# RVC-Project/obs-rvc

Measured on AMD Instinct MI355X. Metric: audio frames/sec (10 ms hops of new input, 160 ms chunks @16 kHz), higher is better.
Workload: dtype f32; 1 GPU; BASELINE configs[1]: 1 stream(s)/GPU, ContentVec v2-768 + RMVPE + NSF-HiFiGAN v2-48k, retrieval off, preset full; streams_per_gpu=1, streams_total=1, hip_graph=False

## Files before the change

### include/rvc_mi355x_debug.h

```cpp
#ifndef RVC_MI355X_DEBUG_H
#define RVC_MI355X_DEBUG_H
#include "rvc_mi355x.h"
#ifdef __cplusplus
extern "C" {
#endif

int rvc_debug_option(const char *name, const char *value);
int rvc_debug_stamps(rvc_engine *e, char *buf, size_t cap);
int rvc_debug_last_plan(rvc_engine *e, int *n_ops);
int rvc_debug_tap(rvc_engine *e, const char *name, int stream, float *out, size_t cap, size_t *n);
int rvc_debug_profile_dump(rvc_engine *e, char *buf, size_t cap);
double rvc_debug_conv_check(rvc_engine *e, int M, int Cin, int KW, int dil, int N, int streams, int pre_act);
double rvc_debug_conv2d_check(rvc_engine *e, int M, int Cin, int H, int W, int streams, int kind, int residual);
double rvc_debug_ln_fold_check(rvc_engine *e, int M, int K, int N, float offset);
typedef struct rvc_debug_layer_spec {
    int form, streams;
    int cin, cout, kw, stride, pad, dil, groups;
    int t_in, t_out, x_halo, y_halo, r_halo;
    int act; float slope; float scale; int accumulate;
    int pre_act; float pre_slope;
    int no_bias, final_out, glu;
    int res;
    int n, kws[4], dils[4], pads[4];
    int x_grouped, res_grouped, y_ws;
} rvc_debug_layer_spec;
int rvc_debug_layer(rvc_engine *e, const rvc_debug_layer_spec *s, const float *w, const float *bias, float *x, float *y, float *r, long long *geo);
typedef struct rvc_debug_op_spec {
    int op, streams;
    int E, heads, T, window, C, H;
    int x_halo, y_halo;
    int reps, graph;
} rvc_debug_op_spec;
int rvc_debug_op(rvc_engine *e, const rvc_debug_op_spec *s, const float *w0, const float *w1, float *x, float *y, int *status, long long *geo);
typedef struct rvc_debug_stream_state {
    float uppower; unsigned stream_id, chunk; int status;
    float cache_pitchf[1024];
} rvc_debug_stream_state;
typedef struct rvc_debug_front_spec {
    int op, streams, graph;
    int n, frame;
    float bn_scale, bn_shift;
    int C, L;
    int Tm, update, shift, cache_start, read_start, R;
    int T, upp, x_halo, f0_num, f0_den;
    float sr, lin_w, lin_b;
    unsigned seed;
} rvc_debug_front_spec;
int rvc_debug_front(rvc_engine *e, const rvc_debug_front_spec *s, const float *w0, const float *w1, float *const *buf, rvc_debug_stream_state *state, long long *geo);
typedef struct rvc_debug_protect_spec {
    int streams, C, R, T, skip_head, ph_ld, cv_ld, graph;
} rvc_debug_protect_spec;
int rvc_debug_protect(rvc_engine *e, const rvc_debug_protect_spec *s, float *phone, const float *cv, const float *pitchf, const double *protect);
typedef struct rvc_debug_post_spec {
    int op, streams, graph;
    int n, frame, hop;
    int sola_len, search;
    int f, skip, copy_begin;
    int rate_in, rate_out, chunk, chunks;
    long long in_bs, out_bs, r_bs, sola_bs, frame_bs, cor_bs, x_bs;
} rvc_debug_post_spec;
int rvc_debug_post(rvc_engine *e, const rvc_debug_post_spec *s, float *const *buf, const float *mix_power, int *offsets);
typedef struct rvc_debug_rm_block_spec {
    int streams, cin, cout, H, W;
    int pool_in, pool_out, y_in_cat, next, rm_fuse;
    int graph, reps;
} rvc_debug_rm_block_spec;
// ... 26 lines not shown
```

### obs_rvc_amd/csrc/debug.hip

```cpp
#include "engine_int.h"
#include "../../include/rvc_mi355x_debug.h"
#include <deque>

namespace {

struct DebugGeo {
    float *base = nullptr; long long g[8] = {0, 0, 0, 0, 0, 0, 0, 1};
    bool live() const { return base && g[0] > 0; }
    void upload(const float *h) const { if (live()) HIPCHK(hipMemcpy(base, h, (size_t)g[0] * 4, hipMemcpyHostToDevice)); }
    void download(float *h) const { if (live()) HIPCHK(hipMemcpy(h, base, (size_t)g[0] * 4, hipMemcpyDeviceToHost)); }
};
DebugGeo debug_geo1(const T1 &t)
{
    DebugGeo q; const size_t gd = t1_guard(t.ld);
    q.base = t.p - gd - t.halo; q.g[0] = (long long)t.B * t.bs + 2 * (long long)gd; q.g[1] = (long long)gd + t.halo; q.g[2] = t.C; q.g[3] = t.T; q.g[4] = t.ld; q.g[5] = t.bs; q.g[6] = t.ld;
    return q;
}
DebugGeo debug_geo2(const T2 &t)
{
    DebugGeo q; const size_t gd = t2_guard(t.ld);
    q.base = t.p - gd - t.ld - 1; q.g[0] = (long long)t.B * t.bs + 2 * (long long)gd; q.g[1] = (long long)gd + t.ld + 1; q.g[2] = t.C; q.g[3] = t.W; q.g[4] = t.ld; q.g[5] = t.bs; q.g[6] = t.cs; q.g[7] = t.H;
    return q;
}
DebugGeo debug_geo_flat(float *p, long long n, int C, int T) { DebugGeo q; q.base = p; q.g[0] = n; q.g[1] = 0; q.g[2] = C; q.g[3] = T; q.g[4] = T; q.g[5] = (long long)C * T; q.g[6] = T; return q; }
// ... 399 lines not shown
        Plan pl; pl.B = B;
        DebugWeights wts;
        T1 x1, y1;
        if (op <= 1) { x1 = make_t1(pl.arena, B, 3 * s->E, s->T, s->x_halo); y1 = make_t1(pl.arena, B, s->E, s->T, s->y_halo); }
        else if (op == 2) x1 = make_t1(pl.arena, B, s->C, s->T, s->x_halo);
        else { x1 = make_t1(pl.arena, B, 6 * s->H, s->T, s->x_halo); y1 = make_t1(pl.arena, B, 2 * s->H, s->T, s->y_halo); }
        const DebugGeo gx = debug_geo1(x1), gy = op == 2 ? DebugGeo() : debug_geo1(y1);
        for (int i = 0; i < 8; i++) { geo[i] = gx.g[i]; geo[8 + i] = gy.g[i]; }
        if (!x) return RVC_OK;
        if ((op != 2 && !y) || (op != 0 && (!w0 || !w1)) || (op == 3 && !status)) throw ShapeError("op buffers");
        gx.upload(x); gy.upload(y);
        int *d_status = nullptr;
        if (op == 0) add_attention(pl, x1, y1, s->heads);
        else if (op == 1) {
            const size_t n = (size_t)(2 * s->window + 1) * (s->E / s->heads);
            float *rk = wts.dev(upload_f(w0, n)), *rv = wts.dev(upload_f(w1, n));
            add_relpos_attention(pl, x1, y1, s->heads, rk, rv, s->window);
        } else if (op == 2) {
            float *g = wts.dev(upload_f(w0, (size_t)s->C)), *b = wts.dev(upload_f(w1, (size_t)s->C));
            add_layernorm(pl, x1, g, b);
        } else {
            const int H = s->H;
            const float *whh_dir[2] = {w0, w0 + (size_t)3 * H * H};
            std::vector<float> wt, wr;
            gru_prep_whh(whh_dir, H, wt, wr);
            float *dwt = wts.dev(upload_f(wt)), *dwr = wts.dev(upload_f(wr)), *bhh = wts.dev(upload_f(w1, (size_t)6 * H));
            d_status = (int *)pl.arena.alloc((size_t)B * sizeof(int));
            HIPCHK(hipMemset(d_status, 0, (size_t)B * sizeof(int)));
            add_gru(pl, x1, y1, H, dwr, dwt, bhh, d_status, 1);
        }
        run_ops(e, pl, s->reps, s->graph != 0);
        gx.download(x); gy.download(y);
        if (d_status) HIPCHK(hipMemcpy(status, d_status, (size_t)B * sizeof(int), hipMemcpyDeviceToHost));
        return RVC_OK;
    });
}

int rvc_debug_front(rvc_engine *e, const rvc_debug_front_spec *s, const float *w0, const float *w1, float *const *buf, rvc_debug_stream_state *state, long long *geo)
{
    return (int)guarded(e, [&]() {
        if (!s || !geo || s->streams < 1 || s->streams > 4096 || s->op < 4 || s->op > 7) throw ShapeError("front spec");
        const int B = s->streams, op = s->op;
        Plan pl; pl.B = B;
        DebugWeights wts;
        Arena &A = pl.arena;
        DebugGeo g[4];
        T1 x1, y1; T2 img; int Tm = 0, R = 0;
        float *f0 = nullptr, *pitchf = nullptr, *mel = nullptr; int *pitch = nullptr;
        if (op == 4) {
            if (s->n < 1 || s->n > (1 << 24) || s->frame < 1 || s->frame > s->n) throw ShapeError("front spec");
            Tm = 1 + s->frame / 160;
            if (Tm > 1024) throw ShapeError("f0 window too long");
            const long long na = (long long)B * s->n + 64;
            g[0] = debug_geo_flat(A.floats((size_t)na), na, 1, s->n);
            mel = A.floats((size_t)B * 128 * Tm); g[1] = debug_geo_flat(mel, (long long)B * 128 * Tm, 128, Tm);
            img = make_t2(A, B, 1, Tm, 128); g[2] = debug_geo2(img);
        } else if (op == 5) {
            if (s->C < 1 || s->C > 4096 || s->L < 10 || s->L > (1 << 22)) throw ShapeError("front spec");
            const long long na = (long long)B * s->L + 64;
            x1.p = A.floats((size_t)na); x1.B = B; x1.C = 1; x1.T = s->L; x1.ld = s->L; x1.halo = 0; x1.bs = s->L;
            g[0] = debug_geo_flat(x1.p, na, 1, s->L);
            y1 = make_t1(A, B, s->C, (s->L - 10) / 5 + 1, 0); g[1] = debug_geo1(y1);
        } else if (op == 6) {
            Tm = s->Tm; R = s->update ? s->R : 0;
            if (Tm < 1 || Tm > 1024 || R < 0 || R > 1024) throw ShapeError("front spec");
            x1 = make_t1(A, B, 360, Tm, 0); g[0] = debug_geo1(x1);
// ... 344 lines not shown
```

### obs_rvc_amd/csrc/engine_int.h

```cpp
#pragma once
#include "../../include/rvc_mi355x.h"
#include "blob.h"
#include "state.hip.h"
#include "formant.hip.h"
#include "f0cond.hip.h"
#include "igemm_launch.h"
#include "dev_raii.h"
#include <hip/hip_ext.h>

#include <algorithm>
#include <atomic>
#include <cmath>
#include <cstdarg>
#include <cstddef>
#include <functional>
#include <map>
#include <memory>
#include <mutex>
#include <string>
#include <tuple>
#include <vector>
#include <thread>

namespace rvc {
// ... 204 lines not shown
    {
        if (!profile) return nullptr;
        if (prof_used == prof.size()) { ProfEvent e; HIPCHK(hipEventCreate(&e.a)); HIPCHK(hipEventCreate(&e.b)); prof.push_back(e); }
        ProfEvent *pe = &prof[prof_used++];
        pe->flops = flops; pe->bytes = bytes; pe->desc = desc; pe->retrieval = retrieval_name != nullptr; pe->name = retrieval_name;
        return pe;
    }
    ~Plan()
    {
        for (float *p : owned_dev) wfree(p);
        if (graph_exec) (void)hipGraphExecDestroy(graph_exec);
        if (ev_done) (void)hipEventDestroy(ev_done);
        for (auto &e : prof) { (void)hipEventDestroy(e.a); (void)hipEventDestroy(e.b); }
    }
};


extern unsigned long long *g_kprobe;
extern int g_last_waves, g_last_wgs, g_ncu;
extern thread_local char g_last_kernel[32];
void queue_igemm(Plan &pl, IgemmP p, int B, const std::vector<int> &koff, const std::vector<PhaseD> &phases, bool final_out = false);
template <class Launch> void queue_gemm_launch(Plan &pl, const char *desc, double flops, int wgs, int waves, bool final_out, const IgemmP &p, Launch launch);
void fill_epilogue(IgemmP &p, const ConvW &cw, const ConvOpts &o);
void add_conv1d(Plan &pl, const ConvW &cw, const T1 &x, const T1 &y, int stride, int pad, int dil, ConvOpts o = ConvOpts());
void add_conv1d_multi(Plan &pl, const std::vector<const ConvW *> &cws, const T1 &x, bool x_grouped, const T1 &y,
                      const std::vector<int> &pads, const std::vector<int> &dils, ConvOpts o = ConvOpts(), bool res_grouped = true);
void add_conv1d_two(Plan &pl, const ConvW &c0, const ConvW &c1, const float *pair_bias, const T1 &x, const T1 &y0, const T1 &y1);
void add_convT1d(Plan &pl, const ConvW &cw, const T1 &x, const T1 &y, int pad, ConvOpts o = ConvOpts());
void add_conv2d(Plan &pl, const ConvW &cw, const T2 &x, const T2 &y, ConvOpts o = ConvOpts());
void add_convT2d(Plan &pl, const ConvW &cw, const T2 &x, const T2 &y, ConvOpts o = ConvOpts());
void add_layernorm(Plan &pl, const T1 &x, const float *g, const float *b);
void add_attention(Plan &pl, const T1 &qkv, const T1 &out, int heads);
void add_relpos_attention(Plan &pl, const T1 &qkv, const T1 &out, int heads, const float *rel_k, const float *rel_v, int window);
void add_gru(Plan &pl, const T1 &gi, const T1 &out, int H, const float *whh, const float *whhT, const float *bhh, int *status, int status_stride);
void add_stamp(Plan &pl, const char *name);
void add_tap(Plan &pl, const char *name, const T1 &t);
void add_tap2(Plan &pl, const char *name, const T2 &t);
void plan_kernel_attrs();
void retrieval_kernel_attrs();

struct DevVec { float *p = nullptr; };
static inline float *dv(const Blob &b, const std::string &name) { const BlobTensor &t = b.t(name); return upload_f(t.data, t.nelem); }

struct ModelCV {
    int conv_dim, embed, heads, ffn, run_layers, pos_k, pos_groups, out_dim;
    int conv_k[7], conv_s[7];
    ConvW conv[7], proj, pos, final_proj;
    float *gn_g, *gn_b, *ln0_g, *ln0_b, *encln_g, *encln_b;
    float *conv0_raw = nullptr;
    struct Layer { ConvW qkv, o, ff1, ff2, qkv_f, ff1_f; float *qkv_wsum = nullptr, *ff1_wsum = nullptr; float *ln1_g, *ln1_b, *ln2_g, *ln2_b; };
    bool has_folded = false;
    ConvW proj_f; float *proj_wsum = nullptr;
    static ConvW fold_ln(const float *w, const float *bias, int M, int K, const float *g, const float *beta, float **wsum_dev);
    std::vector<Layer> layers;
    std::vector<float *> owned;
    size_t weight_bytes = 0;
    explicit ModelCV(const Blob &b);
    ~ModelCV();
    int out_frames(size_t L) const
    {
        long long T = (long long)L;
        for (int i = 0; i < 7; i++) { if (T < conv_k[i]) return 0; T = (T - conv_k[i]) / conv_s[i] + 1; }
        return (int)T;
    }
};

// ... 198 lines not shown
```

### obs_rvc_amd/csrc/model_synth.hip

```cpp
#include "engine_int.h"
#include "synth.hip.h"

namespace rvc {

template <typename T> void glu_pack_rows(const T *w, const float *bias, int H, size_t K, std::vector<float> &wp, std::vector<float> &bp)
{
    if (H % 8 != 0) throw std::runtime_error("GLU-gated layer: channel count must be a multiple of 8");
    wp.resize((size_t)2 * H * K); bp.resize((size_t)2 * H);
    for (int r = 0; r < 2 * H; r++) {
        const int f = r >> 4, kq = (r & 15) >> 2, rr = r & 3;
        const int src = f * 8 + kq * 2 + (rr & 1) + (rr >= 2 ? H : 0);
        for (size_t q = 0; q < K; q++) wp[(size_t)r * K + q] = (float)w[(size_t)src * K + q];
        bp[r] = bias[src];
    }
}
template void glu_pack_rows<float>(const float *, const float *, int, size_t, std::vector<float> &, std::vector<float> &);
template void glu_pack_rows<double>(const double *, const float *, int, size_t, std::vector<float> &, std::vector<float> &);
ModelSY::ModelSY(const Blob &b)
{
    phone_dim = b.icfg("phone_dim"); hidden = b.icfg("hidden"); inter = b.icfg("inter"); filter = b.icfg("filter"); heads = b.icfg("heads");
    enc_layers = b.icfg("enc_layers"); enc_k = b.icfg("enc_k"); window = b.icfg("window"); flow_n = b.icfg("flow_n");
    wn_layers = b.icfg("wn_layers"); wn_k = b.icfg("wn_k"); gin = b.icfg("gin"); up_init = b.icfg("up_init"); n_ups = b.icfg("n_ups");
    n_rb = b.icfg("n_rb"); n_rbd = b.icfg("n_rbd"); sr = b.icfg("sr");
    for (int i = 0; i < n_ups; i++) { up_rate[i] = b.icfg(fmt("up_rate%d", i)); up_kernel[i] = b.icfg(fmt("up_kernel%d", i)); }
// ... 273 lines not shown
std::vector<T1> build_noise_convs(rvc_engine *e, Plan &pl, int B, const T1 &src)
{
    ModelSY &m = *e->sy;
    std::vector<T1> nz;
    int c = m.up_init, Tc = pl.dec_frames();
    for (int i = 0; i < m.n_ups; i++) {
        const int co = c / 2, Tn = Tc * m.up_rate[i];
        T1 t = make_t1(pl.arena, B, co, Tn, 0);
        int sf = 1; for (int q = i + 1; q < m.n_ups; q++) sf *= m.up_rate[q];
        if (i + 1 < m.n_ups) add_conv1d(pl, m.ncs[i], src, t, sf, sf / 2, 1); else add_conv1d(pl, m.ncs[i], src, t, 1, 0, 1);
        nz.push_back(t);
        c = co; Tc = Tn;
    }
    return nz;
}

void build_synth(rvc_engine *e, Plan &pl, int B, const T1 &phone, const T1 &src, float *d_pitchf, int *d_pitch, int src_join_sid,
                        const std::vector<T1> *nz)
{
    ModelSY &m = *e->sy;
    Arena &A = pl.arena;
    const int R = (int)pl.R, H = m.hidden, I = m.inter, F = m.filter, half = I / 2;
    const int HALO = 4;
    if (m.enc_k / 2 > HALO || m.wn_k / 2 > HALO) throw ShapeError("synth kernel sizes exceed the halo");
    T1 z = make_t1(A, B, I, R, HALO), zf = make_t1(A, B, I, R, HALO);
    {
        T1 x = make_t1(A, B, H, R, HALO);
        add_conv1d(pl, m.phone, phone, x, 1, 0, 1);
        {
            dim3 grid((H * R + 255) / 256, B); float *emb = m.pitch_emb; float sq = sqrtf((float)H);
            pl.ops.push_back([=](hipStream_t s) { hipLaunchKernelGGL(embed_pitch_kernel, grid, dim3(256), 0, s, x.p, x.ld, x.bs, emb, d_pitch, H, R, sq); });
        }
        add_tap(pl, "sy.emb", x);
        T1 qkv = make_t1(A, B, 3 * H, R, 0), att = make_t1(A, B, H, R, 0), ff = make_t1(A, B, F, R, HALO);
        const bool fuse_ln = B <= LN_FOLD_MAX_STREAMS && m.has_folded && !pl.plain_plan && !test_opt("RVC_NO_LN_FUSE");
        bool raw = false; const float *raw_g = nullptr, *raw_b = nullptr; float *raw_st = nullptr;
        for (int l = 0; l < m.enc_layers; l++) {
            ModelSY::Layer &Ly = m.layers[l];
            if (raw) { raw_st = A.floats((size_t)2 * R + 16); ConvOpts o; o.ln_wsum = Ly.qkv_wsum; o.ln_stats_out = raw_st; o.ln_rows = H; add_conv1d(pl, Ly.qkv_f, x, qkv, 1, 0, 1, o); }
            else add_conv1d(pl, Ly.qkv, x, qkv, 1, 0, 1);
            add_relpos_attention(pl, qkv, att, m.heads, Ly.rel_k, Ly.rel_v, m.window);
            {
                ConvOpts o; o.res = x.p; o.res_cs = x.ld; o.res_bs = x.bs;
                if (raw) { o.ln_stats_in = raw_st; o.ln_g = raw_g; o.ln_b = raw_b; }
                add_conv1d(pl, Ly.o, att, x, 1, 0, 1, o);
            }
            add_layernorm(pl, x, Ly.ln1_g, Ly.ln1_b);
            { ConvOpts o; o.act = ACT_RELU; add_conv1d(pl, Ly.ff1, x, ff, 1, m.enc_k / 2, 1, o); }
            { ConvOpts o; o.res = x.p; o.res_cs = x.ld; o.res_bs = x.bs; add_conv1d(pl, Ly.ff2, ff, x, 1, m.enc_k / 2, 1, o); }
            if (fuse_ln) { raw = true; raw_g = Ly.ln2_g; raw_b = Ly.ln2_b; }
            else add_layernorm(pl, x, Ly.ln2_g, Ly.ln2_b);
        }
        add_tap(pl, raw ? "sy.enc.raw" : "sy.enc", x);
        static const int wn_max_b = tune_env("RVC_WN_COMPOSE_MAX") ? atoi(tune_env("RVC_WN_COMPOSE_MAX")) : 8;
        const bool wn_composed = B <= wn_max_b && H % 16 == 0 && I == H && !pl.plain_plan && !test_opt("RVC_NO_WN_COMPOSE");
        T1 U[2];
        const int u_z = 16 + H + H * m.wn_layers;
        if (wn_composed) {
            m.compose_flows();
            std::vector<float> ones(R, 1.0f);
            for (int k = 0; k < 2; k++) {
                U[k] = make_t1(A, B, u_z + I, R, HALO);
                for (int bb = 0; bb < B; bb++) HIPCHK(hipMemcpy(U[k].p + (long long)bb * U[k].bs, ones.data(), (size_t)R * sizeof(float), hipMemcpyHostToDevice));
            }
            z = U[0].rows(u_z, I);
        }
        T1 stats = make_t1(A, B, 2 * I, R, 0);
        if (raw) { ConvOpts o; o.ln_wsum = m.proj_wsum; o.ln_rows = H; add_conv1d(pl, m.proj_f, x, stats, 1, 0, 1, o); }
        else add_conv1d(pl, m.proj, x, stats, 1, 0, 1);
        add_tap(pl, "sy.stats", stats);
        {
            dim3 grid(((I * R + 3) / 4 + 255) / 256, B); StreamState *st = e->d_state; CallParams *cp = e->d_cp;
            pl.ops.push_back([=](hipStream_t s) { hipLaunchKernelGGL(prior_sample_kernel, grid, dim3(256), 0, s, stats.p, stats.ld, stats.bs, z.p, z.ld, z.bs, I, R, st, cp); });
        }
        add_tap(pl, "sy.zp", z);
        T1 hs = make_t1(A, B, 2 * H, R, HALO), acts = make_t1(A, B, H, R, 0);
        T1 hh = hs.rows(0, H), skip = hs.rows(H, H);
        for (int fi = m.flow_n - 1; fi >= 0; fi--) {
            ModelSY::Flow &Fw = m.flows[fi];
            const T1 x0 = Fw.flipped ? z.rows(half, half) : z.rows(0, half), x1 = Fw.flipped ? z.rows(0, half) : z.rows(half, half);
// ... 143 lines not shown
```

### obs_rvc_amd/csrc/plan.hip

```cpp
#include "engine_int.h"
#include "plan_ops.hip.h"
#include <chrono>

namespace rvc {

struct TestHook { const char *name; bool planner; };
static const TestHook kTestHooks[] = {
    {"RVC_FORCE_CFG", true}, {"RVC_CONV_TILE", true}, {"RVC_CONV_TILE_KS", true}, {"RVC_NO_LN_FUSE", false}, {"RVC_NO_CONV0_MULTI", false},
    {"RVC_KNN_NO_GEMM", false}, {"RVC_KNN_EXHAUSTIVE", false}, {"RVC_STAMPS", false}, {"RVC_SERIAL_BRANCHES", false}, {"RVC_NO_WN_COMPOSE", false},
    {"RVC_KNN_LOSE_TICKET", false}, {"RVC_FORCE_G2W", true}, {"RVC_F0_XCDS", false}, {"RVC_CONV32S", true}, {"RVC_CONV32S_TILE", true},
    {"RVC_G32L", true}, {"RVC_G32L_TALL", true}, {"RVC_G32L_TAB", true}, {"RVC_CONV32S_BUF", true}, {"RVC_FORCE_CHOICE", true},
    {"RVC_G32L_PANEL", true}, {"RVC_MEAN3", false}, {"RVC_RM_FUSE", false}, {"RVC_G2W_LN", false}, {"RVC_RELPOS_MFMA_MAX", false},
    {"RVC_ATTN_KERNEL", false}, {"RVC_RELPOS_KERNEL", false}, {"RVC_LN_KERNEL", false}, {"RVC_GRU_KERNEL", false}, {"RVC_CONV0_KERNEL", false},
    {"RVC_YIN_CV_ALL_CUS", false}, {"RVC_KNN_WGS", true}, {"RVC_CONV_TILE_MFMA", true}
};
std::atomic<unsigned> g_opt_gen{0};
static std::mutex g_opt_mu;
static std::map<std::string, std::string> g_opts;
static bool is_test_hook(const char *name)
{
    for (const TestHook &h : kTestHooks) if (!strcmp(h.name, name)) return true;
    return false;
}
static const char *opt_lookup(const char *name)
{
    static thread_local std::string buf;
    std::lock_guard<std::mutex> lk(g_opt_mu);
    auto it = g_opts.find(name);
    if (it == g_opts.end()) return nullptr;
    buf = it->second;
    return buf.c_str();
}
#ifdef RVC_TUNING
const char *test_opt(const char *name) { const char *v = opt_lookup(name); return v ? v : getenv(name); }
const char *tune_env(const char *name) { const char *v = opt_lookup(name); return v ? v : getenv(name); }
#else
const char *test_opt(const char *name) { return opt_lookup(name); }
#endif
int test_opt_int(const char *name, int dflt) { const char *v = test_opt(name); return v ? atoi(v) : dflt; }

namespace {
struct WSlab { char *base; size_t size, used; long live; int dev, cls; };
std::mutex g_wslab_mu;
std::vector<WSlab> g_wslabs;
const size_t kWSlabBytes = (size_t)256 << 20, kPlanSlabBytes = (size_t)64 << 20;
void *wmalloc_cls(size_t bytes, int cls)
{
// ... 1156 lines not shown
    } else {
        pl.ops.push_back([=](hipStream_t s) { hipLaunchKernelGGL(attention_kernel, ag, dim3(256), attn_lds, s, ap); });
    }
}

void add_relpos_attention(Plan &pl, const T1 &qkv, const T1 &out, int heads, const float *rel_k, const float *rel_v, int window)
{
    const int B = qkv.B, H = out.C, R = qkv.T, kc = H / heads, Tp = R | 1;
    if (heads < 1 || H % heads || qkv.C != 3 * H || out.T != R || out.B != B || window < 0) throw ShapeError("relative-position attention: inconsistent shapes");
    const size_t attn_lds = attn_valu_lds(kc, R);
    if (attn_lds > 160 * 1024) throw ShapeError("synth attention: return_length too long for the LDS-resident kernel");
    AttnP ap = attn_params(qkv, out, heads);
    ap.rel_k = rel_k; ap.rel_v = rel_v; ap.window = window;
    const size_t small_lds = ((size_t)2 * kc * Tp + 2 * (2 * window + 1) * kc + 4 * kc + 4 * 64) * sizeof(float);
    const int a_tp = R | 1, a_nr = 2 * window + 1, a_jf = (R + 15) / 16, a_pw = (a_nr + 15) / 16 * 16, a_nrp = (a_nr + 3) / 4 * 4;
    const size_t mfma_lds = ((size_t)kc * 16 + 2 * (size_t)kc * a_tp + (size_t)a_pw * kc + (size_t)a_nrp * kc + 16 * a_jf * 16 + 2 * 16 * a_pw + 64) * sizeof(float);
    const bool mfma_ok = R <= 64 && kc % 16 == 0 && mfma_lds <= 160 * 1024, small_ok = R <= 64 && small_lds <= 160 * 1024;
    std::string rule = "valu";
    if (B <= test_opt_int("RVC_RELPOS_MFMA_MAX", 1 << 20) && mfma_ok && !tune_env("RVC_NO_SMALL_ATTN") && !tune_env("RVC_ATTN_VALU") && !tune_env("RVC_NO_SMALL_ATTN_MFMA")) rule = "mfma";
    else if (small_ok && !tune_env("RVC_NO_SMALL_ATTN")) rule = "small";
    const std::string v = op_variant("RVC_RELPOS_KERNEL", "relpos", rule, {{"mfma", mfma_ok}, {"small", small_ok}, {"valu", true}});
    if (v == "mfma") {
        dim3 ag(heads * a_jf, B);
        pl.ops.push_back([=](hipStream_t s) { hipLaunchKernelGGL(relpos_attention_mfma_kernel, ag, dim3(256), mfma_lds, s, ap); });
    } else if (v == "small") {
        dim3 ag(heads * ((R + 3) / 4), B);
        pl.ops.push_back([=](hipStream_t s) { hipLaunchKernelGGL(relpos_attention_small_kernel, ag, dim3(256), small_lds, s, ap); });
    } else {
        dim3 ag(heads * ((R + 15) / 16), B);
        pl.ops.push_back([=](hipStream_t s) { hipLaunchKernelGGL(attention_kernel, ag, dim3(256), attn_lds, s, ap); });
    }
}

void add_gru(Plan &pl, const T1 &gi, const T1 &out, int Hg, const float *whh, const float *whhT, const float *bhh, int *status, int status_stride)
{
    const int B = gi.B, Tm = gi.T;
    if (gi.C != 6 * Hg || out.C != 2 * Hg || out.T != Tm || out.B != B) throw ShapeError("GRU: inconsistent shapes");
    if (3 * Hg > 1024) throw ShapeError("GRU hidden size too large for the single-workgroup recurrence");
    const bool multi_ok = Hg == 256 && B <= 8 && Tm <= 256;
    const std::string rule = multi_ok && !tune_env("RVC_GRU_GENERIC") ? "multi" : "generic";
    const std::string v = op_variant("RVC_GRU_KERNEL", "gru", rule, {{"multi", multi_ok}, {"generic", true}});
    if (v == "multi") {
        GruMultiP gp{}; gp.gi = gi.p; gp.gi_cs = gi.ld; gp.gi_bs = gi.bs; gp.whh = whh; gp.bhh = bhh; gp.out = out.p; gp.o_cs = out.ld; gp.o_bs = out.bs;
        gp.Tm = Tm; gp.status = status; gp.status_stride = status_stride;
        const size_t gbytes = (size_t)B * 2 * 2 * 256 * sizeof(unsigned long long);
        gp.gran = (unsigned long long *)pl.arena.alloc(gbytes);
        const size_t lds3 = (size_t)(256 + 96 + (size_t)Tm * 96) * sizeof(float);
        const dim3 g3(8, 2, B);
        auto next_epoch = std::make_shared<unsigned>(0u);
        auto dirty = std::make_shared<bool>(true);
        pl.ops.push_back([=](hipStream_t s) {
            GruMultiP g2 = gp;
            hipStreamCaptureStatus cs = hipStreamCaptureStatusNone;
            (void)hipStreamIsCapturing(s, &cs);
            if (cs != hipStreamCaptureStatusNone) { HIPCHK(hipMemsetAsync(g2.gran, 0, gbytes, s)); g2.epoch = 0; *dirty = true; }
            else if (*dirty || *next_epoch > 0xFFF00000u) { HIPCHK(hipMemsetAsync(g2.gran, 0, gbytes, s)); g2.epoch = 0; *next_epoch = (unsigned)Tm; *dirty = false; }
            else { g2.epoch = *next_epoch; *next_epoch += (unsigned)Tm; }
            hipLaunchKernelGGL(gru_multi_kernel, g3, dim3(384), lds3, s, g2);
        });
    } else {
        const int threads = (3 * Hg + 63) / 64 * 64;
        const size_t lds = (size_t)4 * Hg * sizeof(float);
        const dim3 grid(2, B);
        pl.ops.push_back([=](hipStream_t s) { hipLaunchKernelGGL(gru_kernel, grid, dim3(threads), lds, s, gi.p, gi.ld, gi.bs, whhT, bhh, out.p, out.ld, out.bs, Hg, Tm); });
    }
}
// ... 30 lines not shown
{
    if (c0.M != c1.M || c0.Kp != c1.Kp || c0.KW != 1 || c1.KW != 1 || c0.Cin != x.C || y0.ld != y1.ld || y0.T != y1.T || y0.bs != y1.bs || y0.C != c0.M || y1.C != c1.M)
        throw ShapeError("conv1d pair: shapes differ");
    IgemmP p{};
    p.x = x.p; p.w = c0.w; p.y = y0.p;
    p.M = c0.M; p.N = y0.T; p.K = c0.Kp;
    p.NW = y0.T; p.x_hs = 0; p.x_ws = 1; p.y_hm = 0; p.y_ws = 1; p.OW = y0.T;
    p.x_bs = x.bs; p.y_bs = y0.bs; p.y_cs = y0.ld; p.y_rs = 0;
    ConvOpts o;
    fill_epilogue(p, c0, o);
    p.bias = pair_bias;
    std::vector<int> koff(c0.Kp, 0);
    for (int ci = 0; ci < c0.Cin; ci++) koff[ci] = ci * x.ld;
    std::vector<PhaseD> ph(2);
    ph[0] = PhaseD{}; ph[1] = PhaseD{};
    ph[0].nchunks = c0.Kp / 16;
    ph[1].w_off = c1.w - c0.w;
    ph[1].nchunks = c1.Kp / 16;
    ph[1].koff_off = 0;
    ph[1].bias_off = c0.M;
    ph[1].act_p1 = ACT_NONE + 1;
    ph[1].y_off = y1.p - y0.p;
    queue_igemm(pl, p, x.B, koff, ph);
}


void plan_kernel_attrs()
{
    HIPCHK(hipFuncSetAttribute((const void *)layernorm_tile_kernel, hipFuncAttributeMaxDynamicSharedMemorySize, 152 * 1024));
    HIPCHK(hipFuncSetAttribute((const void *)attention_kernel, hipFuncAttributeMaxDynamicSharedMemorySize, 160 * 1024));
    HIPCHK(hipFuncSetAttribute((const void *)relpos_attention_small_kernel, hipFuncAttributeMaxDynamicSharedMemorySize, 160 * 1024));
    HIPCHK(hipFuncSetAttribute((const void *)relpos_attention_mfma_kernel, hipFuncAttributeMaxDynamicSharedMemorySize, 160 * 1024));
    HIPCHK(hipFuncSetAttribute((const void *)gru_multi_kernel, hipFuncAttributeMaxDynamicSharedMemorySize, 160 * 1024));
    conv_tile_prepare_device();
    igemm2w_prepare_device();
}

}

extern "C" int rvc_debug_weight_slabs(int device, int *count, size_t *bytes)
{
    int c = 0; size_t b = 0;
    rvc::wslab_info(device, &c, &b);
    if (count) *count = c;
    if (bytes) *bytes = b;
    return 0;
}

extern "C" int rvc_debug_option(const char *name, const char *value)
{
    using namespace rvc;
    if (!name) return -1;
#ifndef RVC_TUNING
    if (!is_test_hook(name)) return -1;
#endif
    std::lock_guard<std::mutex> lk(g_opt_mu);
    if (value) g_opts[name] = value; else g_opts.erase(name);
    if (!strcmp(name, "RVC_KNN_LOSE_TICKET")) g_knn_test_lose.store(value && atoi(value) ? 1 : 0);
    g_opt_gen.fetch_add(1);
    return 0;
}
```

Measured before the change: 8148 frames/s.

## Fuse relpos attention, output projection, residual and layernorm into one kernel

Adds a single-launch kernel for the synthesizer encoder's attention block. It computes relative-position attention with MFMA, the 1x1 output projection with weights held in registers, the optional normalised residual, and the layernorm, all per 16-column tile. Before, this took three or four launches with attention output round-tripping through global memory. The kernel is used by default for one stream on eligible shapes. The cost is heavy register and LDS use in a 768-thread workgroup, and K/V are reloaded by every column tile.

```diff
diff --git a/include/rvc_mi355x_debug.h b/include/rvc_mi355x_debug.h
--- a/include/rvc_mi355x_debug.h
+++ b/include/rvc_mi355x_debug.h
@@ -32,6 +32,13 @@
     int reps, graph;
 } rvc_debug_op_spec;
 int rvc_debug_op(rvc_engine *e, const rvc_debug_op_spec *s, const float *w0, const float *w1, float *x, float *y, int *status, long long *geo);
+typedef struct rvc_debug_relpos_block_spec {
+    int streams, H, heads, T, window;
+    int qkv_halo, x_halo;
+    int res_norm;
+    int reps, graph;
+} rvc_debug_relpos_block_spec;
+int rvc_debug_relpos_block(rvc_engine *e, const rvc_debug_relpos_block_spec *s, const float *const *w, const float *res_stats, float *qkv, float *x, long long *geo);
 typedef struct rvc_debug_stream_state {
     float uppower; unsigned stream_id, chunk; int status;
     float cache_pitchf[1024];
diff --git a/obs_rvc_amd/csrc/debug.hip b/obs_rvc_amd/csrc/debug.hip
--- a/obs_rvc_amd/csrc/debug.hip
+++ b/obs_rvc_amd/csrc/debug.hip
@@ -455,6 +455,34 @@
         run_ops(e, pl, s->reps, s->graph != 0);
         gx.download(x); gy.download(y);
         if (d_status) HIPCHK(hipMemcpy(status, d_status, (size_t)B * sizeof(int), hipMemcpyDeviceToHost));
+        return RVC_OK;
+    });
+}
+
+int rvc_debug_relpos_block(rvc_engine *e, const rvc_debug_relpos_block_spec *s, const float *const *w, const float *res_stats, float *qkv, float *x, long long *geo)
+{
+    return (int)guarded(e, [&]() {
+        if (!s || !geo || s->streams < 1 || s->T < 1 || s->H < 1 || s->heads < 1 || s->H % s->heads || s->window < 0 || s->reps < 1 || s->qkv_halo < 0 || s->x_halo < 0)
+            throw ShapeError("relpos block spec");
+        const int B = s->streams, H = s->H;
+        Plan pl; pl.B = B;
+        DebugWeights wts;
+        T1 q1 = make_t1(pl.arena, B, 3 * H, s->T, s->qkv_halo), x1 = make_t1(pl.arena, B, H, s->T, s->x_halo), att;
+        const DebugGeo gq = debug_geo1(q1), gx = debug_geo1(x1);
+        for (int i = 0; i < 8; i++) { geo[i] = gq.g[i]; geo[8 + i] = gx.g[i]; }
+        if (!qkv) return RVC_OK;
+        if (!x || !w || (s->res_norm && !res_stats)) throw ShapeError("relpos block buffers");
+        for (int i = 0; i < (s->res_norm ? 8 : 6); i++) if (!w[i]) throw ShapeError("relpos block buffers");
+        gq.upload(qkv); gx.upload(x);
+        const size_t nrel = (size_t)(2 * s->window + 1) * (H / s->heads);
+        float *rk = wts.dev(upload_f(w[0], nrel)), *rv = wts.dev(upload_f(w[1], nrel));
+        const ConvW &o = wts.conv(prep_conv(w[2], w[3], H, H, 1, 1));
+        float *g = wts.dev(upload_f(w[4], (size_t)H)), *bt = wts.dev(upload_f(w[5], (size_t)H));
+        float *rg = nullptr, *rb = nullptr, *st = nullptr;
+        if (s->res_norm) { rg = wts.dev(upload_f(w[6], (size_t)H)); rb = wts.dev(upload_f(w[7], (size_t)H)); st = wts.dev(upload_f(res_stats, (size_t)2 * B * s->T)); }
+        add_relpos_block(pl, q1, x1, att, s->heads, rk, rv, s->window, o, g, bt, st, rg, rb);
+        run_ops(e, pl, s->reps, s->graph != 0);
+        gq.download(qkv); gx.download(x);
         return RVC_OK;
     });
 }
diff --git a/obs_rvc_amd/csrc/engine_int.h b/obs_rvc_amd/csrc/engine_int.h
--- a/obs_rvc_amd/csrc/engine_int.h
+++ b/obs_rvc_amd/csrc/engine_int.h
@@ -260,6 +260,9 @@
 void add_layernorm(Plan &pl, const T1 &x, const float *g, const float *b);
 void add_attention(Plan &pl, const T1 &qkv, const T1 &out, int heads);
 void add_relpos_attention(Plan &pl, const T1 &qkv, const T1 &out, int heads, const float *rel_k, const float *rel_v, int window);
+constexpr int RELPOS_BLOCK_MAX_STREAMS = 1;
+void add_relpos_block(Plan &pl, const T1 &qkv, const T1 &x, T1 &att, int heads, const float *rel_k, const float *rel_v, int window, const ConvW &o,
+                      const float *ln_g, const float *ln_b, const float *res_st = nullptr, const float *res_g = nullptr, const float *res_b = nullptr);
 void add_gru(Plan &pl, const T1 &gi, const T1 &out, int H, const float *whh, const float *whhT, const float *bhh, int *status, int status_stride);
 void add_stamp(Plan &pl, const char *name);
 void add_tap(Plan &pl, const char *name, const T1 &t);
diff --git a/obs_rvc_amd/csrc/model_synth.hip b/obs_rvc_amd/csrc/model_synth.hip
--- a/obs_rvc_amd/csrc/model_synth.hip
+++ b/obs_rvc_amd/csrc/model_synth.hip
@@ -329,20 +329,14 @@
             pl.ops.push_back([=](hipStream_t s) { hipLaunchKernelGGL(embed_pitch_kernel, grid, dim3(256), 0, s, x.p, x.ld, x.bs, emb, d_pitch, H, R, sq); });
         }
         add_tap(pl, "sy.emb", x);
-        T1 qkv = make_t1(A, B, 3 * H, R, 0), att = make_t1(A, B, H, R, 0), ff = make_t1(A, B, F, R, HALO);
+        T1 qkv = make_t1(A, B, 3 * H, R, 0), att, ff = make_t1(A, B, F, R, HALO);
         const bool fuse_ln = B <= LN_FOLD_MAX_STREAMS && m.has_folded && !pl.plain_plan && !test_opt("RVC_NO_LN_FUSE");
         bool raw = false; const float *raw_g = nullptr, *raw_b = nullptr; float *raw_st = nullptr;
         for (int l = 0; l < m.enc_layers; l++) {
             ModelSY::Layer &Ly = m.layers[l];
             if (raw) { raw_st = A.floats((size_t)2 * R + 16); ConvOpts o; o.ln_wsum = Ly.qkv_wsum; o.ln_stats_out = raw_st; o.ln_rows = H; add_conv1d(pl, Ly.qkv_f, x, qkv, 1, 0, 1, o); }
             else add_conv1d(pl, Ly.qkv, x, qkv, 1, 0, 1);
-            add_relpos_attention(pl, qkv, att, m.heads, Ly.rel_k, Ly.rel_v, m.window);
-            {
-                ConvOpts o; o.res = x.p; o.res_cs = x.ld; o.res_bs = x.bs;
-                if (raw) { o.ln_stats_in = raw_st; o.ln_g = raw_g; o.ln_b = raw_b; }
-                add_conv1d(pl, Ly.o, att, x, 1, 0, 1, o);
-            }
-            add_layernorm(pl, x, Ly.ln1_g, Ly.ln1_b);
+            add_relpos_block(pl, qkv, x, att, m.heads, Ly.rel_k, Ly.rel_v, m.window, Ly.o, Ly.ln1_g, Ly.ln1_b, raw ? raw_st : nullptr, raw_g, raw_b);
             { ConvOpts o; o.act = ACT_RELU; add_conv1d(pl, Ly.ff1, x, ff, 1, m.enc_k / 2, 1, o); }
             { ConvOpts o; o.res = x.p; o.res_cs = x.ld; o.res_bs = x.bs; add_conv1d(pl, Ly.ff2, ff, x, 1, m.enc_k / 2, 1, o); }
             if (fuse_ln) { raw = true; raw_g = Ly.ln2_g; raw_b = Ly.ln2_b; }
diff --git a/obs_rvc_amd/csrc/plan.hip b/obs_rvc_amd/csrc/plan.hip
--- a/obs_rvc_amd/csrc/plan.hip
+++ b/obs_rvc_amd/csrc/plan.hip
@@ -1,5 +1,6 @@
 #include "engine_int.h"
 #include "plan_ops.hip.h"
+#include "relpos_block.hip.h"
 #include <chrono>
 
 namespace rvc {
@@ -12,7 +13,7 @@
     {"RVC_G32L", true}, {"RVC_G32L_TALL", true}, {"RVC_G32L_TAB", true}, {"RVC_CONV32S_BUF", true}, {"RVC_FORCE_CHOICE", true},
     {"RVC_G32L_PANEL", true}, {"RVC_MEAN3", false}, {"RVC_RM_FUSE", false}, {"RVC_G2W_LN", false}, {"RVC_RELPOS_MFMA_MAX", false},
     {"RVC_ATTN_KERNEL", false}, {"RVC_RELPOS_KERNEL", false}, {"RVC_LN_KERNEL", false}, {"RVC_GRU_KERNEL", false}, {"RVC_CONV0_KERNEL", false},
-    {"RVC_YIN_CV_ALL_CUS", false}, {"RVC_KNN_WGS", true}, {"RVC_CONV_TILE_MFMA", true}
+    {"RVC_YIN_CV_ALL_CUS", false}, {"RVC_KNN_WGS", true}, {"RVC_CONV_TILE_MFMA", true}, {"RVC_RELPOS_BLOCK", false}
 };
 std::atomic<unsigned> g_opt_gen{0};
 static std::mutex g_opt_mu;
@@ -1235,6 +1236,45 @@
     }
 }
 
+void add_relpos_block(Plan &pl, const T1 &qkv, const T1 &x, T1 &att, int heads, const float *rel_k, const float *rel_v, int window, const ConvW &o,
+                      const float *ln_g, const float *ln_b, const float *res_st, const float *res_g, const float *res_b)
+{
+    const int B = qkv.B, H = x.C, R = qkv.T;
+    if (heads < 1 || H % heads || qkv.C != 3 * H || x.T != R || x.B != B || window < 0 || o.Cout != H || o.Cin != H || o.KW != 1 || !o.bias) throw ShapeError("relative-position block: inconsistent shapes");
+    if (res_st && !(res_g && res_b)) throw std::logic_error("normalised residual without scale / shift");
+    const int kc = H / heads;
+    const bool shape_ok = R <= 64 && kc % 16 == 0 && H <= 256 && o.M == H && o.K == H && o.Kp == H && o.nphase == 1 && !o.transposed && qkv.ld >= R && x.ld >= R;
+    const size_t lds = shape_ok ? relpos_block_lds_floats(H, heads, R, window) * sizeof(float) : 0;
+    const bool ok = shape_ok && lds <= 160 * 1024 && !pl.plain_plan;
+    int qb = ok && B <= RELPOS_BLOCK_MAX_STREAMS ? 16 : 0;
+    if (const char *f = test_opt("RVC_RELPOS_BLOCK")) {
+        const std::string v = f;
+        if (v == "0") qb = 0;
+        else if (v == "1") qb = ok ? 16 : 0;
+        else if (v == "8" || v == "16") { if (!ok) throw ShapeError("RVC_RELPOS_BLOCK: the one-launch block is not eligible for this shape"); qb = atoi(f); }
+        else throw ShapeError("RVC_RELPOS_BLOCK: unknown value '" + v + "'");
+    }
+    if (qb) {
+        RelposBlockP bp{};
+        bp.qkv = qkv.p; bp.cs = qkv.ld; bp.bs = qkv.bs; bp.x = x.p; bp.x_cs = x.ld; bp.x_bs = x.bs; bp.rel_k = rel_k; bp.rel_v = rel_v; bp.wo = o.w; bp.bo = o.bias;
+        bp.ln_g = ln_g; bp.ln_b = ln_b; bp.res_st = res_st; bp.res_g = res_g; bp.res_b = res_b; bp.H = H; bp.heads = heads; bp.T = R; bp.window = window;
+        bp.scale = 1.0f / sqrtf((float)kc);
+        const dim3 grid((R + qb - 1) / qb, B);
+        snprintf(g_last_kernel, sizeof g_last_kernel, "rpblock_qb%d", qb);
+        if (qb == 8) pl.ops.push_back([=](hipStream_t s) { hipLaunchKernelGGL((relpos_block_kernel<8>), grid, dim3(RPB_NT), lds, s, bp); });
+        else pl.ops.push_back([=](hipStream_t s) { hipLaunchKernelGGL((relpos_block_kernel<16>), grid, dim3(RPB_NT), lds, s, bp); });
+        return;
+    }
+    if (!att.p) att = make_t1(pl.arena, B, H, R, 0);
+    add_relpos_attention(pl, qkv, att, heads, rel_k, rel_v, window);
+    {
+        ConvOpts co; co.res = x.p; co.res_cs = x.ld; co.res_bs = x.bs;
+        if (res_st) { co.ln_stats_in = res_st; co.ln_g = res_g; co.ln_b = res_b; }
+        add_conv1d(pl, o, att, x, 1, 0, 1, co);
+    }
+    add_layernorm(pl, x, ln_g, ln_b);
+}
+
 void add_gru(Plan &pl, const T1 &gi, const T1 &out, int Hg, const float *whh, const float *whhT, const float *bhh, int *status, int status_stride)
 {
     const int B = gi.B, Tm = gi.T;
@@ -1331,6 +1371,8 @@
     HIPCHK(hipFuncSetAttribute((const void *)relpos_attention_small_kernel, hipFuncAttributeMaxDynamicSharedMemorySize, 160 * 1024));
     HIPCHK(hipFuncSetAttribute((const void *)relpos_attention_mfma_kernel, hipFuncAttributeMaxDynamicSharedMemorySize, 160 * 1024));
     HIPCHK(hipFuncSetAttribute((const void *)gru_multi_kernel, hipFuncAttributeMaxDynamicSharedMemorySize, 160 * 1024));
+    HIPCHK(hipFuncSetAttribute((const void *)relpos_block_kernel<8>, hipFuncAttributeMaxDynamicSharedMemorySize, 160 * 1024));
+    HIPCHK(hipFuncSetAttribute((const void *)relpos_block_kernel<16>, hipFuncAttributeMaxDynamicSharedMemorySize, 160 * 1024));
     conv_tile_prepare_device();
     igemm2w_prepare_device();
 }
diff --git a/obs_rvc_amd/csrc/relpos_block.hip.h b/obs_rvc_amd/csrc/relpos_block.hip.h
--- /dev/null
+++ b/obs_rvc_amd/csrc/relpos_block.hip.h
@@ -0,0 +1,228 @@
+#pragma once
+#include "plan_ops.hip.h"
+
+namespace rvc {
+
+struct RelposBlockP {
+    const float *qkv; int cs; long long bs;
+    float *x; int x_cs; long long x_bs;
+    const float *rel_k, *rel_v;
+    const float *wo, *bo;
+    const float *ln_g, *ln_b;
+    const float *res_st, *res_g, *res_b;
+    int H, heads, T, window;
+    float scale;
+};
+
+constexpr int RPB_NT = 768, RPB_NW = RPB_NT / 64, RPB_AW = 20;
+
+static inline size_t relpos_block_lds_floats(int H, int heads, int T, int window)
+{
+    const int kc = H / heads, TP = T | 1, NR = 2 * window + 1, NRP = (NR + 3) & ~3, SW = (T + 15) / 16 * 16, PW = (NR + 15) / 16 * 16;
+    return (size_t)H * RPB_AW + 2 * (size_t)H * TP + (size_t)PW * kc + (size_t)NRP * kc + (size_t)heads * 16 * (SW + 2 * PW) + 2 * RPB_NW * 16;
+}
+
+struct RpbEpi { float bias[4], res[4], g[4], bt[4]; };
+__device__ __forceinline__ RpbEpi rpb_epi(const RelposBlockP &p, int b, int mt, int kq, int tq, bool ok)
+{
+    RpbEpi e;
+    float mu = 0.f, rs = 1.f;
+    if (p.res_st && ok) { const long long n = (long long)b * p.T + tq; mu = p.res_st[2 * n]; rs = p.res_st[2 * n + 1]; }
+#pragma unroll
+    for (int r = 0; r < 4; r++) {
+        const int row = mt * 16 + kq * 4 + r;
+        e.bias[r] = p.bo[row]; e.g[r] = p.ln_g[row]; e.bt[r] = p.ln_b[row];
+        float xr = ok ? p.x[(long long)b * p.x_bs + (long long)row * p.x_cs + tq] : 0.f;
+        if (p.res_st && ok) xr = (xr - mu) * rs * p.res_g[row] + p.res_b[row];
+        e.res[r] = xr;
+    }
+    return e;
+}
+
+template <int QB>
+static __global__ __launch_bounds__(RPB_NT) void relpos_block_kernel(RelposBlockP p)
+{
+    extern __shared__ __attribute__((aligned(16))) float smem[];
+    constexpr int NT = RPB_NT, NW = RPB_NW, AW = RPB_AW;
+    const int H = p.H, heads = p.heads, kc = H / heads, T = p.T, TP = T | 1, Wd = p.window, NR = 2 * Wd + 1, NRP = (NR + 3) & ~3;
+    const int JF = (T + 15) >> 4, SW = JF * 16, RF = (NR + 15) >> 4, PW = RF * 16, MT = H >> 4;
+    const int b = blockIdx.y, col0 = blockIdx.x * QB, nq = T - col0 < QB ? T - col0 : QB;
+    float *q = smem, *att = smem, *kk = q + H * AW, *vv = kk + H * TP, *rk = vv + H * TP, *rv = rk + PW * kc;
+    float *Sx = rv + NRP * kc, *P = Sx + heads * 16 * SW, *Ssk = P + heads * 16 * PW, *red = Ssk + heads * 16 * PW;
+    const float *base = p.qkv + (long long)b * p.bs;
+    const int tid = threadIdx.x, lane = tid & 63, wave = tid >> 6, li = lane & 15, kq = lane >> 4;
+    const f32x4 zero4 = {0.f, 0.f, 0.f, 0.f};
+    f32x4 wreg[16];
+    RpbEpi epi[2];
+    {
+        const f32x4 *wp = reinterpret_cast<const f32x4 *>(p.wo) + (long long)wave * MT * 64 + lane;
+#pragma unroll
+        for (int c = 0; c < 16; c++) wreg[c] = (wave < MT && c < MT) ? wp[c * 64] : zero4;
+        if (wave < MT) epi[0] = rpb_epi(p, b, wave, kq, col0 + li, li < nq);
+    }
+    const int tsh = T <= 32 ? 5 : 6, tmask = (1 << tsh) - 1;
+    constexpr int KV_IT = 8, RT_IT = 4, Q_IT = 4;
+    const int kv_n = H << tsh, rk_n = PW * kc, rv_n = NRP * kc, rt_n = NR * kc, q_n = H * 16;
+    {
+        float kr[KV_IT], vr[KV_IT], rkr[RT_IT], rvr[RT_IT], qr[Q_IT];
+#pragma unroll
+        for (int u = 0; u < Q_IT; u++) {
+            const int idx = tid + u * NT, d = idx >> 4, c = idx & 15;
+            qr[u] = (idx < q_n && c < nq) ? base[(long long)d * p.cs + col0 + c] * p.scale : 0.f;
+        }
+#pragma unroll
+        for (int u = 0; u < KV_IT; u++) {
+            const int idx = tid + u * NT, d = idx >> tsh, t = idx & tmask;
+            const bool ok = idx < kv_n && t < T;
+            kr[u] = ok ? base[(long long)(H + d) * p.cs + t] : 0.f;
+            vr[u] = ok ? base[(long long)(2 * H + d) * p.cs + t] : 0.f;
+        }
+#pragma unroll
+        for (int u = 0; u < RT_IT; u++) {
+            const int j = tid + u * NT;
+            rkr[u] = j < rt_n ? p.rel_k[j] : 0.f;
+            rvr[u] = j < rt_n ? p.rel_v[j] : 0.f;
+        }
+#pragma unroll
+        for (int u = 0; u < Q_IT; u++) { const int idx = tid + u * NT; if (idx < q_n) q[idx] = qr[u]; }
+#pragma unroll
+        for (int u = 0; u < KV_IT; u++) {
+            const int idx = tid + u * NT, d = idx >> tsh, t = idx & tmask;
+            if (idx < kv_n && t < TP) { kk[d * TP + t] = kr[u]; vv[d * TP + t] = vr[u]; }
+        }
+#pragma unroll
+        for (int u = 0; u < RT_IT; u++) {
+            const int j = tid + u * NT;
+            if (j < rk_n) rk[j] = rkr[u];
+            if (j < rv_n) rv[j] = rvr[u];
+        }
+    }
+    for (int idx = tid + Q_IT * NT; idx < q_n; idx += NT) { const int d = idx >> 4, c = idx & 15; q[idx] = c < nq ? base[(long long)d * p.cs + col0 + c] * p.scale : 0.f; }
+    for (int idx = tid + KV_IT * NT; idx < kv_n; idx += NT) {
+        const int d = idx >> tsh, t = idx & tmask;
+        if (t < TP) { kk[d * TP + t] = t < T ? base[(long long)(H + d) * p.cs + t] : 0.f; vv[d * TP + t] = t < T ? base[(long long)(2 * H + d) * p.cs + t] : 0.f; }
+    }
+    for (int j = tid + RT_IT * NT; j < rk_n; j += NT) rk[j] = j < rt_n ? p.rel_k[j] : 0.f;
+    for (int j = tid + RT_IT * NT; j < rv_n; j += NT) rv[j] = j < rt_n ? p.rel_v[j] : 0.f;
+    __syncthreads();
+    for (int it = wave; it < heads * (JF + RF); it += NW) {
+        const int h = it / (JF + RF), f2 = it - h * (JF + RF);
+        const bool is_p = f2 >= JF;
+        const int f = is_p ? f2 - JF : f2;
+        f32x4 a0 = zero4, a1 = zero4;
+        const float *qa = q + h * kc * 16 + kq * 16 + li;
+        const float *bb = is_p ? rk + (f * 16 + li) * kc + kq : kk + (h * kc + kq) * TP + f * 16 + li;
+        const int bst = is_p ? 4 : 4 * TP;
+        for (int ks = 0; ks + 1 < kc / 4; ks += 2) {
+            a0 = __builtin_amdgcn_mfma_f32_16x16x4f32(qa[ks * 64], bb[ks * bst], a0, 0, 0, 0);
+            a1 = __builtin_amdgcn_mfma_f32_16x16x4f32(qa[(ks + 1) * 64], bb[(ks + 1) * bst], a1, 0, 0, 0);
+        }
+        if ((kc / 4) & 1) a0 = __builtin_amdgcn_mfma_f32_16x16x4f32(qa[(kc / 4 - 1) * 64], bb[(kc / 4 - 1) * bst], a0, 0, 0, 0);
+        a0 += a1;
+        float *dst = is_p ? P + h * 16 * PW + f * 16 : Sx + h * 16 * SW + f * 16;
+        const int dw = is_p ? PW : SW;
+#pragma unroll
+        for (int r = 0; r < 4; r++) dst[(kq * 4 + r) * dw + li] = a0[r];
+    }
+    __syncthreads();
+    for (int h = tid >> 8; h < heads; h += NT / 256) {
+        const int i = (tid & 255) >> 4, gi = col0 + i;
+        float *Sr = Sx + h * 16 * SW + i * SW, *Kr = Ssk + h * 16 * PW + i * PW;
+        const float *Pr = P + h * 16 * PW + i * PW;
+        const bool own = i < nq;
+        float mx = -INFINITY;
+        if (own) {
+            for (int j = li; j < T; j += 16) {
+                float a = Sr[j];
+                const int r = j - gi;
+                if (r >= -Wd && r <= Wd) a += Pr[r + Wd];
+                Sr[j] = a; mx = fmaxf(mx, a);
+            }
+        }
+#pragma unroll
+        for (int o = 8; o >= 1; o >>= 1) mx = fmaxf(mx, __shfl_xor(mx, o, 16));
+        float sum = 0.f;
+        if (own) for (int j = li; j < T; j += 16) { const float ex = expf(Sr[j] - mx); Sr[j] = ex; sum += ex; }
+#pragma unroll
+        for (int o = 8; o >= 1; o >>= 1) sum += __shfl_xor(sum, o, 16);
+        const float inv = 1.0f / sum;
+        for (int j = li; j < SW; j += 16) Sr[j] = (own && j < T) ? Sr[j] * inv : 0.f;
+        for (int r = li; r < PW; r += 16) { const int j = gi + r - Wd; Kr[r] = (own && r < NR && j >= 0 && j < T) ? Sr[j] : 0.f; }
+    }
+    __syncthreads();
+    for (int it = wave; it < MT; it += NW) {
+        const int h = it / (kc / 16), cf = it - h * (kc / 16);
+        f32x4 a0 = zero4, a1 = zero4;
+        const float *va = vv + (it * 16 + li) * TP + kq, *sb = Sx + h * 16 * SW + li * SW + kq;
+        for (int ks = 0; ks < (T + 3) / 4; ks++) a0 = __builtin_amdgcn_mfma_f32_16x16x4f32(va[ks * 4], sb[ks * 4], a0, 0, 0, 0);
+        const float *ra = rv + kq * kc + cf * 16 + li, *kb = Ssk + h * 16 * PW + li * PW + kq;
+        for (int ks = 0; ks < NRP / 4; ks++) a1 = __builtin_amdgcn_mfma_f32_16x16x4f32(ra[ks * 4 * kc], kb[ks * 4], a1, 0, 0, 0);
+        a0 += a1;
+#pragma unroll
+        for (int r = 0; r < 4; r++) att[(it * 16 + kq * 4 + r) * AW + li] = a0[r];
+    }
+    __syncthreads();
+    float v[2][4];
+#pragma unroll
+    for (int ps = 0; ps < 2; ps++) {
+        const int mt = wave + ps * NW;
+#pragma unroll
+        for (int r = 0; r < 4; r++) v[ps][r] = 0.f;
+        if (mt < MT) {
+            if (ps) {
+                const f32x4 *wp = reinterpret_cast<const f32x4 *>(p.wo) + (long long)mt * MT * 64 + lane;
+#pragma unroll
+                for (int c = 0; c < 16; c++) wreg[c] = c < MT ? wp[c * 64] : zero4;
+                epi[1] = rpb_epi(p, b, mt, kq, col0 + li, li < nq);
+            }
+            f32x4 acc = zero4;
+            const float *ab = att + kq * 4 * AW + li;
+#pragma unroll
+            for (int c = 0; c < 16; c++) {
+                if (c < MT) {
+#pragma unroll
+                    for (int j = 0; j < 4; j++) acc = __builtin_amdgcn_mfma_f32_16x16x4f32(wreg[c][j], ab[(c * 16 + j) * AW], acc, 0, 0, 0);
+                }
+            }
+#pragma unroll
+            for (int r = 0; r < 4; r++) v[ps][r] = (acc[r] + epi[ps].bias[r]) + epi[ps].res[r];
+        }
+    }
+    float s = (v[0][0] + v[0][1]) + (v[0][2] + v[0][3]);
+    if (wave + NW < MT) s += (v[1][0] + v[1][1]) + (v[1][2] + v[1][3]);
+    s += __shfl_xor(s, 16, 64); s += __shfl_xor(s, 32, 64);
+    if (lane < 16) red[wave * 16 + li] = s;
+    __syncthreads();
+    float mean = 0.f;
+#pragma unroll
+    for (int w = 0; w < NW; w++) mean += red[w * 16 + li];
+    mean /= (float)H;
+    float qd = 0.f;
+#pragma unroll
+    for (int ps = 0; ps < 2; ps++)
+        if (wave + ps * NW < MT) {
+#pragma unroll
+            for (int r = 0; r < 4; r++) { const float d = v[ps][r] - mean; qd += d * d; }
+        }
+    qd += __shfl_xor(qd, 16, 64); qd += __shfl_xor(qd, 32, 64);
+    if (lane < 16) red[(NW + wave) * 16 + li] = qd;
+    __syncthreads();
+    float var = 0.f;
+#pragma unroll
+    for (int w = 0; w < NW; w++) var += red[(NW + w) * 16 + li];
+    var /= (float)H;
+    const float inv = 1.0f / sqrtf(var + 1e-5f);
+    if (li < nq) {
+        float *xb = p.x + (long long)b * p.x_bs + col0 + li;
+#pragma unroll
+        for (int ps = 0; ps < 2; ps++) {
+            const int mt = wave + ps * NW;
+            if (mt < MT) {
+#pragma unroll
+                for (int r = 0; r < 4; r++) xb[(long long)(mt * 16 + kq * 4 + r) * p.x_cs] = (v[ps][r] - mean) * inv * epi[ps].g[r] + epi[ps].bt[r];
+            }
+        }
+    }
+}
+
+}
```

Result: no change. 8153 frames/s, median of 3 (+0.1%).
